# roahmlab/koopman-realizations

Hardware: AMD Instinct MI355X
Metric: EDMD snapshot-pairs/sec (bilinear fit, 3-link arm, poly-3) (higher is better)
Workload: dtype f64

## Files before the change

### koopman-realizations_amd/csrc/kp_context.hip

```cpp
#include <algorithm>
#include <cmath>
#include <cstring>
#include <mutex>

#include "kp_internal.h"

static std::mutex g_err_mu;
static std::string g_err;

void kp_set_global_error(const std::string& s) {
  std::lock_guard<std::mutex> l(g_err_mu);
  g_err = s;
}

void* kp_ctx::workspace(int slot, size_t bytes) {
  if (ws_bytes[slot] >= bytes && ws[slot]) return ws[slot];
  if (ws[slot]) (void)hipFree(ws[slot]);
  ws[slot] = nullptr;
  ws_bytes[slot] = 0;
  size_t want = bytes + bytes / 4 + 256;
  if (hipMalloc(&ws[slot], want) != hipSuccess) return nullptr;
  ws_bytes[slot] = want;
  return ws[slot];
}
// ... 50 lines not shown
  (void)kp_flush_grams(c);
  (void)kp_comm_destroy(c);
  (void)hipSetDevice(c->device);
  kp_stage_destroy(c);
  (void)hipStreamSynchronize(c->stream);
  if (c->stream2) (void)hipStreamSynchronize(c->stream2);
  for (int i = 0; i < 21; ++i)
    if (c->ws[i]) (void)hipFree(c->ws[i]);
  if (c->sticky_info) (void)hipFree(c->sticky_info);
  if (c->pin_small) (void)hipHostFree(c->pin_small);
  if (c->pin_scratch) (void)hipHostFree(c->pin_scratch);
  if (c->ev_gram_done) (void)hipEventDestroy(c->ev_gram_done);
  if (c->ev_pad_done) (void)hipEventDestroy(c->ev_pad_done);
  if (c->ev_pad_done2) (void)hipEventDestroy(c->ev_pad_done2);
  if (c->ev_main_done) (void)hipEventDestroy(c->ev_main_done);
  if (c->ev_solve0) (void)hipEventDestroy(c->ev_solve0);
  if (c->ev_solve1) (void)hipEventDestroy(c->ev_solve1);
  if (c->stream2) (void)hipStreamDestroy(c->stream2);
  if (c->Kres) (void)hipFree(c->Kres);
  if (c->GC) (void)hipFree(c->GC);
  for (int i = 0; i < 6; ++i)
    if (c->evp[i]) (void)hipEventDestroy(c->evp[i]);
  for (int i = 0; i < 2 * 64; ++i)
    if (c->ring[i]) (void)hipEventDestroy(c->ring[i]);
  for (int i = 0; i < 64; ++i)
    if (c->ring_red[i]) (void)hipEventDestroy(c->ring_red[i]);
  (void)hipEventDestroy(c->ev0);
  (void)hipEventDestroy(c->ev1);
  (void)hipStreamDestroy(c->stream);
  kp_traj_pool_free(c);
  kp_host_free_all(c);
  delete c;
  return KP_OK;
}

extern "C" int kp_device_count(int* count) {
  if (!count) return KP_ERR_ARG;
  int n = 0;
  if (hipGetDeviceCount(&n) != hipSuccess) {
    (void)hipGetLastError();
    n = 0;
  }
  *count = n;
  return KP_OK;
}

extern "C" const char* kp_last_error(const kp_ctx* c) {
  if (c) return c->err.c_str();
  std::lock_guard<std::mutex> l(g_err_mu);
  static thread_local std::string copy;
  copy = g_err;
  return copy.c_str();
}

extern "C" int kp_device_info(const kp_ctx* c, char* name, int name_len, int* num_cu, int64_t* hbm) {
  if (!c) return KP_ERR_ARG;
  if (name && name_len > 0) {
    std::strncpy(name, c->name.c_str(), (size_t)name_len - 1);
    name[name_len - 1] = 0;
  }
  if (num_cu) *num_cu = c->num_cu;
  if (hbm) *hbm = c->hbm_bytes;
  return KP_OK;
}

void* kp_pinned_scratch(kp_ctx* ctx, size_t bytes) {
  if (ctx->pin_scratch_bytes >= bytes) return ctx->pin_scratch;
  if (ctx->pin_scratch) {
    (void)hipStreamSynchronize(ctx->stream);
    (void)hipHostFree(ctx->pin_scratch);
  }
  ctx->pin_scratch = nullptr;
  ctx->pin_scratch_bytes = 0;
  const size_t cap = (bytes + 4095) & ~(size_t)4095;
  if (hipHostMalloc(&ctx->pin_scratch, cap, hipHostMallocDefault) != hipSuccess) {
    ctx->pin_scratch = nullptr;
    return nullptr;
  }
  ctx->pin_scratch_bytes = cap;
  return ctx->pin_scratch;
}

extern "C" int kp_timer_get(const kp_ctx* c, int which, double* ms) {
  if (!c || !ms || which < 0 || which >= 15) return KP_ERR_ARG;
  *ms = c->timers[which];
  return KP_OK;
}

extern "C" void* kp_stream(const kp_ctx* c) { return c ? (void*)c->stream : nullptr; }


static int upload(kp_ctx* ctx, void** dst, const void* src, size_t bytes) {
  *dst = nullptr;
  if (bytes == 0) return KP_OK;
  KP_HIP(ctx, hipMalloc(dst, bytes));
  KP_HIP(ctx, hipMemcpy(*dst, src, bytes, hipMemcpyHostToDevice));
  return KP_OK;
}

extern "C" int kp_basis_desc_dims(const kp_basis_desc* d, int* nvars_out, int* nfull_out, int* N_out, int* W_out) {
  if (!d || d->nzeta < 1 || d->m < 0 || d->model_type < 0 || d->model_type > 2 || d->n_blocks < 0 ||
      (d->n_blocks && (!d->block_type || !d->block_count)))
    return KP_ERR_ARG;
  const int nvars = d->nzeta + (d->model_type == KP_MODEL_NONLINEAR ? d->m : 0);
  double nf = nvars + 1.0;
  for (int b = 0; b < d->n_blocks; ++b) {
    const int c = d->block_count[b];
    if (c < 0) return KP_ERR_ARG;
    switch (d->block_type[b]) {
      case KP_BLOCK_POLY: case KP_BLOCK_HERMITE: case KP_BLOCK_FOURIER_SPARSER: case KP_BLOCK_GAUSSIAN: nf += c; break;
      case KP_BLOCK_FOURIER: nf += std::pow((double)(2 * c + 1), (double)nvars) - 1.0; break;
      default: return KP_ERR_ARG;
    }
    if (nf > 1e6) return KP_ERR_ARG;
  }
  const int nfull = (int)std::llround(nf);
  const int N = d->k_pcs > 0 ? d->k_pcs + nvars + 1 : nfull;
  if (nvars_out) *nvars_out = nvars;
  if (nfull_out) *nfull_out = nfull;
  if (N_out) *N_out = N;
  if (W_out) *W_out = d->model_type == KP_MODEL_BILINEAR ? N * (d->m + 1) : d->model_type == KP_MODEL_LINEAR ? N + d->m : N;
  return KP_OK;
}

extern "C" int kp_basis_create(kp_ctx* ctx, const kp_basis_desc* d, kp_basis** out) {
  if (!ctx || !d || !out) return KP_ERR_ARG;
  *out = nullptr;
  KP_HIP(ctx, hipSetDevice(ctx->device));
  if (d->model_type < 0 || d->model_type > 2) return ctx->fail(KP_ERR_ARG, "kp_basis_create: model_type");
  if (d->nzeta < 1 || d->m < 0) return ctx->fail(KP_ERR_ARG, "kp_basis_create: nzeta/m");
  int nvars = d->nzeta + (d->model_type == KP_MODEL_NONLINEAR ? d->m : 0);
  if (nvars > KP_MAX_VARS) return ctx->fail(KP_ERR_ARG, "kp_basis_create: too many variables (max 32)");
  std::vector<ColDesc> cols;
  for (int i = 0; i < nvars; ++i) cols.push_back({COL_VAR, i, 0, 0});
  int n_mono = 0, n_gauss = 0, max_deg = 1, fourier_deg = 0;
  for (int b = 0; b < d->n_blocks; ++b) {
    int cnt = d->block_count[b];
    if (cnt < 0) return ctx->fail(KP_ERR_ARG, "kp_basis_create: negative block count");
    switch (d->block_type[b]) {
      case KP_BLOCK_POLY:
        if (cnt && !d->poly_exps) return ctx->fail(KP_ERR_ARG, "kp_basis_create: poly_exps is NULL");
        for (int i = 0; i < cnt; ++i) {
          int deg = 0;
          for (int v = 0; v < nvars; ++v) deg += d->poly_exps[(size_t)(n_mono + i) * nvars + v];
          if (deg > max_deg) max_deg = deg;
          uint32_t pk[2] = {0, 0};
          if (nvars <= 8)
            for (int v = 0; v < nvars; ++v) pk[v >> 2] |= (uint32_t)d->poly_exps[(size_t)(n_mono + i) * nvars + v] << (8 * (v & 3));
          cols.push_back({COL_MONO, n_mono + i, (int32_t)pk[0], (int32_t)pk[1]});
        }
        n_mono += cnt;
        break;
      case KP_BLOCK_FOURIER: {
        if (cnt < 1) return ctx->fail(KP_ERR_ARG, "kp_basis_create: fourier degree < 1");
        double nf = std::pow((double)(2 * cnt + 1), (double)nvars);
        if (nf > 1e6) return ctx->fail(KP_ERR_ARG, "kp_basis_create: fourier block too large");
        int total = (int)std::llround(nf);
        for (int i = 1; i < total; ++i) {
          uint32_t pk = 0;
          if (nvars <= 8 && 2 * cnt + 1 <= 16) {
            int idx = i;
            for (int v = nvars - 1; v >= 0; --v) {
              pk |= (uint32_t)(idx % (2 * cnt + 1)) << (4 * v);
              idx /= 2 * cnt + 1;
            }
          }
          cols.push_back({COL_FOURIER, i, cnt, (int32_t)pk});
// ... 380 lines not shown
```

### koopman-realizations_amd/csrc/kp_gram3.hip

```cpp
#include <algorithm>
#include <cstdlib>
#include <type_traits>
#include <vector>

#include "kp_internal.h"

#ifndef KP_RAW_STEP
#define KP_RAW_STEP 1
#endif
#define KT3 8
#define NF3 3
#define RS3 240
#define YOFF3 96
#define ZOFF3 192
#define WOFF3 196
#define SOFF3 208
#define NIDMAX3 144
#define PST3 10
#define POWBUF3 (PST3 * NIDMAX3)
#define PSIBUF3 (KT3 * RS3)
#define PSI03 (2 * POWBUF3)
#define LDS3_DOUBLES (PSI03 + 2 * PSIBUF3)
#define PCS03 LDS3_DOUBLES
#define PCSMAX3 32
// ... 507 lines not shown
    default: run_tiles(std::integral_constant<int, NQ>{}); break;
  }

  double* dst = a.part + (((size_t)split * a.njobs + job) * NQ) * NWT * 64 + lane;
#pragma unroll
  for (int q = 0; q < NQ; ++q)
#pragma unroll
    for (int w = 0; w < NWT; ++w) dst[(q * NWT + w) * 64] = acc[q][w];
}

__global__ __launch_bounds__(1024) void kp_gram3_reduce_kernel(const double* __restrict__ part, int nsplit, int njobs, int NQ, int NWT,
                                                              int BM, const uint32_t* __restrict__ desc, int G4, int N, int W,
                                                              double* __restrict__ G, double* __restrict__ C, int tup,
                                                              const uint32_t* __restrict__ dst_off, const uint32_t* __restrict__ dst) {
  const int idx = blockIdx.x;
  int w = idx % NWT;
  const int jq = idx / NWT, q = jq % NQ, job = jq / NQ;
  const int l = threadIdx.x & 63, wv = threadIdx.x >> 6, nwv = blockDim.x >> 6;
  __shared__ double red[16][64];
  const size_t per_split = (size_t)njobs * NQ * NWT * 64;
  const double* src = part + (size_t)blockIdx.y * nsplit * per_split + (size_t)idx * 64 + l;
  G += (size_t)blockIdx.y * 2 * W * W;
  C += (size_t)blockIdx.y * 2 * W * W;
  double s0 = 0.0, s1 = 0.0, s2 = 0.0, s3 = 0.0;
  int p = wv;
  for (; p + 3 * nwv < nsplit; p += 4 * nwv) {
    const double v0 = src[(size_t)p * per_split], v1 = src[(size_t)(p + nwv) * per_split];
    const double v2 = src[(size_t)(p + 2 * nwv) * per_split], v3 = src[(size_t)(p + 3 * nwv) * per_split];
    s0 += v0; s1 += v1; s2 += v2; s3 += v3;
  }
  for (; p < nsplit; p += nwv) s0 += src[(size_t)p * per_split];
  red[wv][l] = (s0 + s1) + (s2 + s3);
  __syncthreads();
  if (wv) return;
  double s = red[0][l];
  for (int v = 1; v < nwv; ++v) s += red[v][l];
  const uint32_t* jd = desc + (size_t)job * (1 + NQ);
  const int ga = q < (int)((jd[0] >> 16) & 255u) ? (int)(jd[0] & 255u) : (int)((jd[0] >> 8) & 255u);
  int gsel = (l >> 2) & 3;
  if (tup) {
    const int b = gsel;
    gsel = 2 * (w & 1) + (b & 1);
    w = (w & ~1) + (b >> 1);
  }
  const int gb = (int)((jd[1 + q] >> (8 * gsel)) & 255u);
  if (gb >= 2 * G4) return;
  int wa = 0, wb = 0, cnt = 0;
  for (int x = 0; x <= BM; ++x)
    for (int y = x; y <= BM; ++y) {
      if (cnt == w) { wa = x; wb = y; }
      ++cnt;
    }
  const int ia = 4 * ga + (l >> 4);
  if (ia >= N) return;
  if (gb < G4 && dst_off) {
    const int e = (jq * 4 + gsel) * 16 + (l >> 4) * 4 + (l & 3);
    for (uint32_t k = dst_off[e]; k < dst_off[e + 1]; ++k) {
      const uint32_t d = dst[k];
      const size_t di = d & 0xffffu, dj = d >> 16;
      const size_t r1 = (size_t)wa * N + di, c1 = (size_t)wb * N + dj;
      const size_t r2 = (size_t)wb * N + di, c2 = (size_t)wa * N + dj;
      G[c1 * W + r1] = s; G[r1 * W + c1] = s;
      G[c2 * W + r2] = s; G[r2 * W + c2] = s;
    }
  } else if (gb < G4) {
    const int jb = 4 * gb + (l & 3);
    if (jb >= N) return;
    if (ga == gb && ia > jb) return;
    const size_t r1 = (size_t)wa * N + ia, c1 = (size_t)wb * N + jb;
    const size_t r2 = (size_t)wb * N + ia, c2 = (size_t)wa * N + jb;
    G[c1 * W + r1] = s; G[r1 * W + c1] = s;
    G[c2 * W + r2] = s; G[r2 * W + c2] = s;
  } else {
    const int jb = 4 * (gb - G4) + (l & 3);
    if (jb >= N) return;
    C[((size_t)wb * N + jb) * W + (size_t)wa * N + ia] = s;
    C[((size_t)wa * N + jb) * W + (size_t)wb * N + ia] = s;
  }
}

struct kp_gram3_plan {
  int G4 = 0, nq = 0, njobs = 0, nsuper = 0;
  int wpw = 4;
  uint32_t* desc = nullptr;
  uint32_t* dst_off = nullptr;
  uint32_t* dst = nullptr;
  kp_gram3_plan* cover = nullptr;
  bool cover_tried = false;
};

void kp_gram3_plan_free(kp_gram3_plan* p) {
  if (!p) return;
  kp_gram3_plan_free(p->cover);
  if (p->desc) (void)hipFree(p->desc);
  if (p->dst_off) (void)hipFree(p->dst_off);
  if (p->dst) (void)hipFree(p->dst);
  delete p;
}

static hipError_t plan3_upload(uint32_t** dev, const std::vector<uint32_t>& host) {
  hipError_t e = hipMalloc((void**)dev, std::max<size_t>(host.size(), 1) * 4);
  if (e == hipSuccess && !host.empty()) e = hipMemcpy(*dev, host.data(), host.size() * 4, hipMemcpyHostToDevice);
  return e;
}

static int make_plan3(kp_ctx* ctx, int N, int nwt, int nq_cap, kp_gram3_plan** out, int wpw = 4, int nq_force = 0) {
  kp_gram3_plan* p = new kp_gram3_plan();
  p->wpw = wpw;
  const int G4 = (N + 3) / 4;
  p->G4 = G4;
  size_t maxq = 0;
  const std::vector<std::vector<int>> rows = gram3_circulant_rows(G4, &maxq);
  Gram3JobsHost jobs;
  gram3_pack_rows(rows, G4, nwt, nq_cap, maxq, wpw, nq_force, &jobs);
  p->nq = jobs.nq;
  p->njobs = jobs.njobs;
  p->nsuper = jobs.njobs / wpw;
  hipError_t e = plan3_upload(&p->desc, jobs.desc);
  if (e != hipSuccess) {
    kp_gram3_plan_free(p);
    return ctx->fail(KP_ERR_HIP, std::string("kp_fit_gram: plan upload: ") + hipGetErrorString(e));
  }
  *out = p;
  return KP_OK;
}

static bool gram3_tup(int bm) {
  static const bool off = getenv("KP_GRAM3_NOTUP") != nullptr;
  return bm >= 2 && !off;
}

template <int NQ, int BM, bool PCS, bool EXT = false, bool PRE = false, bool TUP = false>
static hipError_t launch3c(const Gram3Args& a, int grid, size_t lds, hipStream_t st) {
  static KpLdsCache lds_cache;
  {
    const size_t lds_max = (size_t)(LDS3_DOUBLES + (PCS ? LDS3_PCS_DOUBLES : 0) + (EXT ? LDS3_GAUSS_DOUBLES : 0)) * sizeof(double);
    hipError_t e = kp_ensure_lds(lds_cache, (const void*)kp_gram3_kernel<NQ, BM, PCS, EXT, PRE, TUP>, lds_max);
    if (e != hipSuccess) return e;
  }
  hipLaunchKernelGGL((kp_gram3_kernel<NQ, BM, PCS, EXT, PRE, TUP>), dim3(grid), dim3(256), lds, st, a);
  return hipGetLastError();
}

template <int NQ, int BM, bool PCS, bool EXT = false, bool PRE = false>
static hipError_t launch3b(const Gram3Args& a, int grid, size_t lds, hipStream_t st) {
  if constexpr (BM >= 2) {
    if (gram3_tup(BM)) return launch3c<NQ, BM, PCS, EXT, PRE, true>(a, grid, lds, st);
  }
  return launch3c<NQ, BM, PCS, EXT, PRE, false>(a, grid, lds, st);
}

template <int NQ>
static hipError_t launch3(const Gram3Args& a, int bm, int grid, size_t lds, hipStream_t st) {
  if (a.pre) {
    switch (bm) {
      case 1: return launch3b<NQ, 1, false, false, true>(a, grid, lds, st);
      case 2: return launch3b<NQ, 2, false, false, true>(a, grid, lds, st);
      default: return launch3b<NQ, 3, false, false, true>(a, grid, lds, st);
    }
  }
  if (a.pcs) {
    if constexpr (NQ <= 4) {
      switch (bm) {
        case 1: return launch3b<NQ, 1, true>(a, grid, lds, st);
        case 2: return launch3b<NQ, 2, true>(a, grid, lds, st);
        default: return launch3b<NQ, 3, true>(a, grid, lds, st);
      }
    } else {
      return hipErrorInvalidValue;
    }
  }
  if (a.df > 0 || a.ng > 0) {
    switch (bm) {
      case 1: return launch3b<NQ, 1, false, true>(a, grid, lds, st);
      case 2: return launch3b<NQ, 2, false, true>(a, grid, lds, st);
      default: return launch3b<NQ, 3, false, true>(a, grid, lds, st);
    }
  }
  switch (bm) {
    case 1: return launch3b<NQ, 1, false>(a, grid, lds, st);
    case 2: return launch3b<NQ, 2, false>(a, grid, lds, st);
    default: return launch3b<NQ, 3, false>(a, grid, lds, st);
  }
}

static bool gram3_ext(const kp_basis* basis) {
  const BasisDev& b = basis->dev;
  return basis->fast_ext && (basis->ext_df > 0 || basis->ext_ng > 0) && b.k_pcs == 0 && basis->ext_ng <= GAUSSMAX3 &&
         (basis->ext_ng == 0 || b.nzeta <= GNZMAX3) && !getenv("KP_NO_GRAM3_EXT");
}

static bool gram3_prelift(const kp_basis* basis) {
  static const bool off = getenv("KP_GRAM3_NO_PRELIFT") != nullptr;
  const BasisDev& b = basis->dev;
  if (off) return false;
  if ((b.N + 3) / 4 > 14) return false;
  if (b.k_pcs > 0) return b.k_pcs <= 32 && basis->fast && b.nzeta * basis->pow_depth <= 24;
  return gram3_ext(basis) && b.nzeta <= 16 && b.nzeta * (basis->ext_Dp + 2 * basis->ext_df) + basis->ext_ng + 1 <= 64;
}

bool kp_gram3_applicable(const kp_basis* basis) {
  const BasisDev& b = basis->dev;
  if (getenv("KP_NO_GRAM3")) return false;
  if (2 * b.nfull + (b.m + 1) * (b.m + 2) / 2 - 1 > 192) return false;
  if (gram3_ext(basis))
    return b.model_type == KP_MODEL_BILINEAR && basis->ext_max_factors <= NF3 && b.nfull <= YOFF3 && b.m >= 1 && b.m <= 3 &&
           2 * (b.nzeta + b.m) * KT3 <= 256 &&
           2 * (b.nzeta + b.m) * (basis->ext_Dp + 2 * basis->ext_df) + 1 + 2 * basis->ext_ng <= NIDMAX3;
  if (b.k_pcs > 0 && (b.k_pcs > PCSMAX3 || b.N != b.nzeta + b.k_pcs + 1 || getenv("KP_NO_GRAM3_PCS"))) return false;
  return b.model_type == KP_MODEL_BILINEAR && basis->fast && basis->max_factors <= NF3 && b.nfull <= YOFF3 && basis->pow_depth <= 4 &&
         b.m >= 1 && b.m <= 3 && (2 * (b.nzeta + b.m) + 1) * KT3 <= 256 && 2 * (b.nzeta + b.m) * 4 + 4 <= NIDMAX3;
}

static bool gram6_on() {
  static const bool on = getenv("KP_GRAM6") != nullptr;
  return on;
}

static int gram3_plan(kp_ctx* ctx, kp_basis* basis) {
  if (basis->plan3) return KP_OK;
  const BasisDev& b = basis->dev;
  const int N = b.N, BM = b.m, NWT = (BM + 1) * (BM + 2) / 2;
  static const int ext_cap = [] { const char* e = getenv("KP_GRAM3_EXT_NQ"); return e ? atoi(e) : 4; }();
  const bool g6 = gram6_on() && BM == 3 && b.k_pcs == 0 && !gram3_ext(basis) && kp_gram6_serves(7, (N + 3) / 4);
  return g6 ? make_plan3(ctx, N, NWT, 7, &basis->plan3, 8, 7)
            : make_plan3(ctx, N, NWT, b.k_pcs > 0 ? 4 : gram3_ext(basis) ? ext_cap : 6, &basis->plan3);
}

static int gram3_cover_mode() {
  static const int v = [] { const char* e = getenv("KP_GRAM3_COVER"); return e ? std::min(2, std::max(0, atoi(e))) : 1; }();
  return v;
}

static int gram3_cover_plan(kp_ctx* ctx, kp_basis* basis, kp_gram3_plan** out) {
  kp_gram3_plan& circ = *basis->plan3;
  *out = nullptr;
  if (!circ.cover_tried) {
    circ.cover_tried = true;
    const BasisDev& b = basis->dev;
    const int N = b.N, NWT = (b.m + 1) * (b.m + 2) / 2;
    if (circ.wpw != 4 || b.k_pcs != 0 || gram3_ext(basis) || !basis->fast || b.nfull != N || (int)basis->h_recipes.size() != N) return KP_OK;
    Gram3CoverHost cov;
    if (!gram3_cover_build(basis->h_recipes.data(), N, basis->pow_depth, NWT, 6, circ.wpw, &cov) || cov.jobs.njobs >= circ.njobs) return KP_OK;
    kp_gram3_plan* p = new kp_gram3_plan();
    p->G4 = circ.G4;
    p->nq = cov.jobs.nq;
    p->njobs = cov.jobs.njobs;
    p->nsuper = cov.jobs.njobs / circ.wpw;
    p->cover_tried = true;
    hipError_t e = plan3_upload(&p->desc, cov.jobs.desc);
    if (e == hipSuccess) e = plan3_upload(&p->dst_off, cov.dst_off);
    if (e == hipSuccess) e = plan3_upload(&p->dst, cov.dst);
    if (e != hipSuccess) {
      kp_gram3_plan_free(p);
      circ.cover_tried = false;
      return ctx->fail(KP_ERR_HIP, std::string("kp_fit_gram: plan upload: ") + hipGetErrorString(e));
    }
    circ.cover = p;
  }
  *out = circ.cover;
  return KP_OK;
}

static int gram3_plan_for(kp_ctx* ctx, kp_basis* basis, bool deferred, kp_gram3_plan** out) {
  int rc = gram3_plan(ctx, basis);
  if (rc) return rc;
  *out = basis->plan3;
  if (gram3_cover_mode() == 2 || (gram3_cover_mode() == 1 && deferred)) {
    kp_gram3_plan* cov = nullptr;
    rc = gram3_cover_plan(ctx, basis, &cov);
    if (rc) return rc;
    if (cov) *out = cov;
  }
  return KP_OK;
}

static int64_t gram3_slots(const kp_ctx* ctx, const kp_gram3_plan& plan, int* ncu_out = nullptr, int* wgpcu_out = nullptr) {
  int ncu = ctx->num_cu > 0 ? ctx->num_cu : 256;
  int wg_per_cu = plan.wpw == 8 ? 1 : 2;
  if (const char* ov = getenv("KP_GRAM3_WGPCU")) wg_per_cu = std::max(1, atoi(ov));
  if (ncu_out) *ncu_out = ncu;
  if (wgpcu_out) *wgpcu_out = wg_per_cu;
  return (int64_t)std::max(8, ncu - ctx->reserve_cus) * wg_per_cu;
}

bool kp_gram3_groupable(kp_ctx* ctx, const kp_basis* basis_c, const kp_snapshots* s) {
  kp_basis* basis = const_cast<kp_basis*>(basis_c);
  const BasisDev& b = basis->dev;
  if (!(kp_gram3_applicable(basis) && b.k_pcs == 0 && !gram3_ext(basis) && !gram6_on() && s->nzeta == b.nzeta && s->m == b.m)) return false;
  kp_gram3_plan* plan = nullptr;
  if (gram3_plan_for(ctx, basis, true, &plan) != KP_OK || plan->wpw == 8) return false;
  static const int64_t max_kps = [] { const char* e = getenv("KP_GRAM_GROUP_MAX_KPS"); return e ? (int64_t)atoll(e) : (int64_t)512; }();
  const int64_t ktiles = (s->Ns + KT3 - 1) / KT3, nsplit = std::max<int64_t>(1, gram3_slots(ctx, *plan) / plan->nsuper);
  return (ktiles + nsplit - 1) / nsplit < max_kps;
}

static int gram3_launch_n(kp_ctx* ctx, const kp_basis* basis_c, const kp_snapshots* const* ss, int n, double* GC_dev, bool cover) {
  kp_basis* basis = const_cast<kp_basis*>(basis_c);
  const BasisDev& b = basis->dev;
  const kp_snapshots* s = ss[0];
  if (n < 1 || n > KP_GRAM_GROUP_MAX) return ctx->fail(KP_ERR_ARG, "kp_fit_gram: bad group size");
  for (int f = 0; f < n; ++f)
    if (ss[f]->nzeta != b.nzeta || ss[f]->m != b.m || ss[f]->Ns != s->Ns) return ctx->fail(KP_ERR_ARG, "kp_fit_gram: snapshot/basis dimension mismatch");
  const int W = b.W, N = b.N;
  const int BM = b.m, NWT = (BM + 1) * (BM + 2) / 2;
  kp_gram3_plan* planp = nullptr;
  {
    int rc = gram3_plan_for(ctx, basis, cover, &planp);
    if (rc) return rc;
  }
  kp_gram3_plan& plan = *planp;
  const int nfull4 = (b.nfull + 3) / 4 * 4;
  const bool ext = gram3_ext(basis);
  
  int64_t ktiles = (s->Ns + KT3 - 1) / KT3;
  int ncu, wg_per_cu;
  const int64_t slots = gram3_slots(ctx, plan, &ncu, &wg_per_cu);
  int nsplit = (int)std::max<int64_t>(1, std::min<int64_t>(ktiles, slots / plan.nsuper / n > 0 ? slots / plan.nsuper / n : 1));
  int kps = (int)((ktiles + nsplit - 1) / nsplit);
  if (kps < 1) kps = 1;
  nsplit = (int)std::max<int64_t>(1, (ktiles + kps - 1) / kps);
  size_t per_split = (size_t)plan.njobs * plan.nq * NWT * 64;
  const size_t part_bytes = ((size_t)n * nsplit * per_split * 8 + 255) & ~(size_t)255;
  if (gram3_cover_mode() != 0) {
    kp_gram3_plan* cov = nullptr;
    int rc = gram3_cover_plan(ctx, basis, &cov);
    if (rc) return rc;
  }
// ... 24 lines not shown
  if (pre && !ext && !basis->d_pcsT) {
    if (hipMalloc(&basis->d_pcsT, (size_t)b.nfull * 32 * 8) != hipSuccess) return ctx->fail(KP_ERR_HIP, "kp_fit_gram: out of device memory");
    KP_HIP(ctx, kp_gram3_pcs_transpose_launch(b.pcs, b.nfull, b.k_pcs, (double*)basis->d_pcsT, ctx->stream));
  }
  const size_t lds = (size_t)(LDS3_DOUBLES + (b.k_pcs > 0 && !pre ? 2 * nfull4 * 16 : 0) + (ext && !pre ? LDS3_GAUSS_DOUBLES : 0)) * sizeof(double);

  Gram3Args a;
  a.b = b;
  a.alpha = s->alpha;
  a.beta = s->beta;
  a.u = s->u;
  a.Ns = s->Ns;
  a.G4 = plan.G4;
  a.nsuper = plan.nsuper;
  a.ktiles_per_split = kps;
  a.D = ext ? basis->ext_Dp + 2 * basis->ext_df : basis->pow_depth;
  a.recipes = (const uint32_t*)(ext ? basis->d_recipes_ext : basis->d_recipes);
  a.Dp = ext ? basis->ext_Dp : basis->pow_depth;
  a.df = ext ? basis->ext_df : 0;
  a.ng = ext ? basis->ext_ng : 0;
  a.centres = b.centres;
  a.desc = plan.desc;
  a.part = part;
  a.njobs = plan.njobs;
  a.pcs = b.k_pcs > 0 && !pre ? b.pcs : nullptr;
  a.nfull4 = nfull4;
  a.pre = pre_buf;
  a.pre_rl = pre_rl;
  a.nsplit_fit = nsplit;
  for (int f = 0; f < n; ++f) a.grp[f] = Gram3Src{ss[f]->alpha, ss[f]->beta, ss[f]->u};
  const int grid = plan.nsuper * nsplit * n;
  const bool pipelined = ctx->reduce_stream || ctx->ring_timing;
  if (!pipelined) KP_HIP(ctx, hipEventRecord(ctx->ev0, ctx->stream));
  hipEvent_t ev_start = ctx->evp[0], ev_end = ctx->evp[1];
  const bool timed = !ctx->ring_timing || (ctx->ring_group && n > 1) || (ctx->ring_skip++ & 3) == 0;
  hipEvent_t ev_red = nullptr;
  if (pipelined && timed) {
    ev_start = ctx->ring[2 * ctx->ring_pos];
    ev_end = ctx->ring[2 * ctx->ring_pos + 1];
    ctx->ring_members[ctx->ring_pos] = n;
    ctx->ring_has_red[ctx->ring_pos] = false;
    if (ctx->ring_timing && ctx->ring_group && n > 1) {
      ev_red = ctx->ring_red[ctx->ring_pos];
      ctx->ring_has_red[ctx->ring_pos] = ev_red != nullptr;
    }
    ctx->ring_pos = (ctx->ring_pos + 1) % 64;
    if (ctx->ring_n < 64) ++ctx->ring_n;
  }
  if (timed) KP_HIP(ctx, hipEventRecord(ev_start, ctx->stream));
  hipError_t e;
  if (pre && ext)
    KP_HIP(ctx, kp_gram3_prelift_ext_launch(BM, s->alpha, s->beta, s->u, s->Ns, ktiles * KT3, b.nzeta, basis->ext_Dp, basis->ext_df, basis->ext_ng, b.nfull, plan.G4,
                                            (const uint32_t*)basis->d_recipes_ext, b.centres, pre_buf, pre_rl, ctx->stream));
  else if (pre)
    KP_HIP(ctx, kp_gram3_prelift_launch(BM, s->alpha, s->beta, s->u, s->Ns, ktiles * KT3, b.nzeta, basis->pow_depth, b.nfull, b.k_pcs, N, plan.G4,
                                        (const uint32_t*)basis->d_recipes, (const double*)basis->d_pcsT, pre_buf, pre_rl, ctx->stream));
  if (plan.wpw == 8) e = kp_gram6_launch_kernel(a, plan.nq, grid, ctx->stream);
  else switch (plan.nq) {
    case 1: e = launch3<1>(a, BM, grid, lds, ctx->stream); break;
    case 2: e = launch3<2>(a, BM, grid, lds, ctx->stream); break;
    case 3: e = launch3<3>(a, BM, grid, lds, ctx->stream); break;
    case 4: e = launch3<4>(a, BM, grid, lds, ctx->stream); break;
    case 5: e = launch3<5>(a, BM, grid, lds, ctx->stream); break;
    default: e = launch3<6>(a, BM, grid, lds, ctx->stream); break;
  }
  KP_HIP(ctx, e);
  if (timed) KP_HIP(ctx, hipEventRecord(ev_end, ctx->stream));
  hipStream_t rs = ctx->stream;
  if (ctx->reduce_stream) {
    rs = ctx->reduce_stream;
    KP_HIP(ctx, hipStreamWaitEvent(rs, ev_end, 0));
    KP_HIP(ctx, hipEventRecord(ctx->evp[4], rs));
    ctx->solve_chained = true;
  }
  ctx->reduce_timed_from = ctx->reduce_stream ? 4 : 1;
  hipLaunchKernelGGL(kp_gram3_reduce_kernel, dim3(plan.njobs * plan.nq * NWT, n), dim3(nsplit >= 128 ? 1024 : nsplit >= 32 ? 512 : 256), 0, rs, part, nsplit, plan.njobs,
                     plan.nq, NWT, BM, plan.desc, plan.G4, N, W, GC_dev, GC_dev + (size_t)W * W, plan.wpw != 8 && gram3_tup(BM) ? 1 : 0, plan.dst_off, plan.dst);
  KP_HIP(ctx, hipGetLastError());
  if (ev_red) KP_HIP(ctx, hipEventRecord(ev_red, rs));
  if (!pipelined) KP_HIP(ctx, hipEventRecord(ctx->ev1, rs));
  if (!ctx->ring_timing) KP_HIP(ctx, hipEventRecord(ctx->evp[2], rs));
  ctx->gram_flops_per_pair = (double)W * (W + 1) + 2.0 * W * W;
  ctx->timers[10] = (double)plan.njobs * plan.nq * NWT * 128.0 + (b.k_pcs > 0 && !pre ? (double)plan.nsuper * nfull4 * 128.0 : 0.0);
  return KP_OK;
}

int kp_gram3_launch(kp_ctx* ctx, const kp_basis* basis, const kp_snapshots* s, double* GC_dev, bool cover) { return gram3_launch_n(ctx, basis, &s, 1, GC_dev, cover); }

int kp_gram3_launch_group(kp_ctx* ctx, const kp_basis* basis, const kp_snapshots* const* ss, int n, double* GC_dev) {
  return gram3_launch_n(ctx, basis, ss, n, GC_dev, true);
}


__global__ __launch_bounds__(256) void kp_gram3_linear_gather_kernel(const double* __restrict__ GCb, int N, int m, int Wb, double* __restrict__ GC) {
  const int W = N + m;
  const int e = blockIdx.x * 256 + threadIdx.x;
  if (e >= 2 * W * W) return;
  const int which = e / (W * W), r = e - which * W * W, i = r % W, j = r / W;
  const int bi = i < N ? i : (i - N + 1) * N + N - 1, bj = j < N ? j : (j - N + 1) * N + N - 1;
  GC[e] = GCb[(size_t)which * Wb * Wb + (size_t)bj * Wb + bi];
}

static kp_basis* gram3_shadow(const kp_basis* basis_c) {
  kp_basis* basis = const_cast<kp_basis*>(basis_c);
  if (!basis->shadow_bil) {
    kp_basis* sh = new kp_basis(*basis);
    sh->dev.model_type = KP_MODEL_BILINEAR;
    sh->dev.W = sh->dev.N * (sh->dev.m + 1);
    sh->plan = nullptr; sh->plan2 = nullptr; sh->plan3 = nullptr; sh->plan5 = nullptr; sh->shadow_bil = nullptr;
    sh->d_pcsT = nullptr;
    basis->shadow_bil = sh;
  }
  return basis->shadow_bil;
}

void kp_gram3_shadow_free(kp_basis* basis) {
  if (!basis) return;
  if (basis->shadow_bil) {
    kp_gram3_plan_free(basis->shadow_bil->plan3);
    if (basis->shadow_bil->d_pcsT) (void)hipFree(basis->shadow_bil->d_pcsT);
    delete basis->shadow_bil;
    basis->shadow_bil = nullptr;
  }
  if (basis->shadow_full) {
    kp_gram_plan_free(basis->shadow_full->plan);
    kp_gram2_plan_free(basis->shadow_full->plan2);
    kp_gram5_plan_free(basis->shadow_full->plan5);
    delete basis->shadow_full;
    basis->shadow_full = nullptr;
  }
}

bool kp_gram3_linear_applicable(const kp_basis* basis) {
  const BasisDev& b = basis->dev;
  if (b.model_type != KP_MODEL_LINEAR || b.k_pcs <= 0 || b.m < 1 || getenv("KP_NO_GRAM3_LINEAR")) return false;
  return kp_gram3_applicable(gram3_shadow(basis));
}

int kp_gram3_linear_launch(kp_ctx* ctx, const kp_basis* basis, const kp_snapshots* s, double* GC_dev) {
  kp_basis* sh = gram3_shadow(basis);
  const int N = basis->dev.N, m = basis->dev.m, W = basis->dev.W, Wb = sh->dev.W;
  double* tmp = (double*)ctx->workspace(10, (size_t)2 * Wb * Wb * 8);
  if (!tmp) return ctx->fail(KP_ERR_HIP, "kp_fit_gram: out of device memory");
  hipStream_t rs = ctx->reduce_stream ? ctx->reduce_stream : ctx->stream;
  int rc = kp_gram3_launch(ctx, sh, s, tmp);
  if (rc) return rc;
  hipLaunchKernelGGL(kp_gram3_linear_gather_kernel, dim3((2 * W * W + 255) / 256), dim3(256), 0, rs, tmp, N, m, Wb, GC_dev);
  KP_HIP(ctx, hipGetLastError());
  ctx->gram_flops_per_pair = (double)W * (W + 1) + 2.0 * W * W;
  return KP_OK;
}


struct CongT { int nvars, k, nfull, N, W, Wf; const double* pcs; };
__device__ __forceinline__ int cong_unit(const CongT& t, int j) {
  if (j < t.nvars) return j;
  if (j < t.nvars + t.k) return -1;
  if (j == t.N - 1) return t.nfull - 1;
  return t.nfull + (j - t.N);
}
__global__ __launch_bounds__(256) void kp_cong_right_kernel(const double* __restrict__ GCf, CongT t, double* __restrict__ R) {
  const int e = blockIdx.x * 256 + threadIdx.x;
  if (e >= t.Wf * t.W) return;
  const int i = e % t.Wf, j = e / t.Wf;
  const double* M = GCf + (size_t)blockIdx.y * t.Wf * t.Wf;
  const int u = cong_unit(t, j);
// ... 77 lines not shown
```

### koopman-realizations_amd/csrc/kp_gram3_cover.h

```cpp
#pragma once
#include <algorithm>
#include <cstdint>
#include <cstdlib>
#include <map>
#include <utility>
#include <vector>

struct Gram3JobsHost {
  int nq = 0, njobs = 0, nquads = 0;
  std::vector<uint32_t> desc;
};

inline std::vector<std::vector<int>> gram3_circulant_rows(int G4, size_t* maxq) {
  std::vector<std::vector<int>> rows(G4);
  *maxq = 0;
  for (int g = 0; g < G4; ++g) {
    for (int d = 0; d <= G4 / 2; ++d) {
      if (d > 0 && 2 * d == G4 && g >= G4 / 2) continue;
      rows[g].push_back((g + d) % G4);
    }
    for (int h = 0; h < G4; ++h) rows[g].push_back(G4 + h);
    *maxq = std::max(*maxq, (rows[g].size() + 3) / 4);
  }
  return rows;
// ... 104 lines not shown

  std::vector<std::vector<int>> rows(G4);
  for (auto& p : chosen)
    if (p.first == p.second) rows[p.first].push_back(p.second);
  std::vector<std::pair<int, int>> off;
  for (auto& p : chosen)
    if (p.first != p.second) off.push_back(p);
  std::sort(off.begin(), off.end());
  auto quads_of = [&](size_t s) { return (s + G4 + 3) / 4; };
  for (auto& p : off) {
    const size_t la = rows[p.first].size(), lb = rows[p.second].size();
    const size_t ca = quads_of(la + 1) - quads_of(la), cb = quads_of(lb + 1) - quads_of(lb);
    const bool to_b = cb < ca || (cb == ca && lb < la);
    rows[to_b ? p.second : p.first].push_back(to_b ? p.first : p.second);
  }
  size_t minq = ~(size_t)0;
  for (int g = 0; g < G4; ++g) {
    for (int h = 0; h < G4; ++h) rows[g].push_back(G4 + h);
    minq = std::min(minq, (rows[g].size() + 3) / 4);
  }
  gram3_pack_rows(rows, G4, nwt, nq_cap, minq, wpw, 0, &out->jobs);
  out->npairs = (int)chosen.size();
  out->nmonos = nm;

  const Gram3JobsHost& J = out->jobs;
  const int nq = J.nq;
  std::vector<int> src(nm, -1);
  std::vector<int> tgroups((size_t)G4 * G4, 0);
  for (int job = 0; job < J.njobs; ++job) {
    const uint32_t* jd = &J.desc[(size_t)job * (1 + nq)];
    const int a0 = (int)(jd[0] & 255u), a1 = (int)((jd[0] >> 8) & 255u), qs = (int)((jd[0] >> 16) & 255u);
    if (a0 >= G4 || a1 >= G4) return false;
    for (int q = 0; q < nq; ++q) {
      const int ga = q < qs ? a0 : a1;
      for (int k = 0; k < 4; ++k) {
        const int gb = (int)((jd[1 + q] >> (8 * k)) & 255u);
        if (gb > 2 * G4) return false;
        if (gb >= G4) {
          if (gb < 2 * G4) ++tgroups[(size_t)ga * G4 + gb - G4];
          continue;
        }
        for (int r = 0; r < 4; ++r)
          for (int c = 0; c < 4; ++c) {
            const int i = 4 * ga + r, j = 4 * gb + c;
            if (i >= N || j >= N) continue;
            int& s = src[mono[(size_t)i * N + j]];
            if (s < 0) s = ((job * nq + q) * 4 + k) * 16 + 4 * r + c;
          }
      }
    }
  }
  for (int t : tgroups)
    if (t != 1) return false;
  const int nel = J.njobs * nq * 64;
  std::vector<uint32_t> cnt(nel + 1, 0);
  for (int i = 0; i < N; ++i)
    for (int j = i; j < N; ++j) {
      const int s = src[mono[(size_t)i * N + j]];
      if (s < 0) return false;
      ++cnt[s + 1];
    }
  for (int e = 0; e < nel; ++e) cnt[e + 1] += cnt[e];
  out->dst_off = cnt;
  out->dst.assign(cnt[nel], 0);
  std::vector<uint32_t> fill(cnt.begin(), cnt.end() - 1);
  for (int i = 0; i < N; ++i)
    for (int j = i; j < N; ++j) out->dst[fill[src[mono[(size_t)i * N + j]]]++] = (uint32_t)i | ((uint32_t)j << 16);
  if ((size_t)cnt[nel] != (size_t)N * (N + 1) / 2) return false;
  for (int e = 0; e < nel; ++e) {
    if (cnt[e] == cnt[e + 1]) continue;
    const int c = e & 3, r = (e >> 2) & 3, k = (e >> 4) & 3, jq = e >> 6, q = jq % nq, job = jq / nq;
    const uint32_t* jd = &J.desc[(size_t)job * (1 + nq)];
    const int ga = q < (int)((jd[0] >> 16) & 255u) ? (int)(jd[0] & 255u) : (int)((jd[0] >> 8) & 255u);
    const int gb = (int)((jd[1 + q] >> (8 * k)) & 255u);
    const int i = 4 * ga + r, j = 4 * gb + c;
    if (gb >= G4 || i >= N || j >= N) return false;
    for (uint32_t d = cnt[e]; d < cnt[e + 1]; ++d) {
      const int di = (int)(out->dst[d] & 0xffffu), dj = (int)(out->dst[d] >> 16);
      if (di > dj || dj >= N || mono[(size_t)di * N + dj] != mono[(size_t)i * N + j]) return false;
    }
  }
  return true;
}
```

### koopman-realizations_amd/csrc/kp_internal.h

```cpp
#pragma once
#include <hip/hip_runtime.h>
#include <stdint.h>
#include <atomic>
#include <mutex>
#include <string>
#include <utility>
#include <vector>

#include "koopman_hip.h"

#define KP_MAX_VARS 32
#define KP_GRAM_GROUP_MAX 8

void kp_set_global_error(const std::string& s);
void kp_traj_device_blocks(kp_traj* t, double** blocks);
struct kp_comm_state;

struct kp_stage;

struct kp_ctx {
  int device = 0;
  kp_stage* stage = nullptr;
  std::vector<void*> host_blocks;
  std::vector<std::pair<void*, size_t>> traj_pool;
  std::mutex host_mu;
  hipStream_t stream = nullptr;
  hipEvent_t ev0 = nullptr, ev1 = nullptr;
  hipEvent_t evp[6] = {nullptr};
  hipStream_t stream2 = nullptr;
  hipEvent_t ev_gram_done = nullptr, ev_pad_done = nullptr, ev_pad_done2 = nullptr, ev_solve0 = nullptr, ev_solve1 = nullptr;
  bool pad_pending = false, pad_pending2 = false, async_pending = false;
  int gc_flip = 0;
  int kring_cap = 128;
  int async_count = 0;
  bool batch_closed = true;
  bool kres_is_ring = false;
  const void* pend_basis = nullptr;
  int64_t pend_Ns = 0;
  int pend_W = 0;
  int pend_solves = 0, pend_first = 0;
  bool ring_timing = false;
  unsigned ring_skip = 0;
  const kp_snapshots* pend_grams[KP_GRAM_GROUP_MAX] = {};
  int pend_ngrams = 0;
  const kp_basis* pend_gram_basis = nullptr;
  double* pend_gram_gc = nullptr;
  bool ring_group = false;
  kp_comm_state* comm = nullptr;
  std::atomic<bool> comm_abandoned{false};
  bool gc_preloaded = false;
  bool reduce_grams = false;
  hipStream_t reduce_stream = nullptr;
  hipEvent_t ev_main_done = nullptr;
  hipEvent_t ring[2 * 64] = {};
  int ring_pos = 0, ring_n = 0;
  hipEvent_t ring_red[64] = {};
  int ring_members[64] = {};
  bool ring_has_red[64] = {};
  bool solve_chained = false;
  int part_flip = 0;
  int reduce_timed_from = 1;
  int* sticky_info = nullptr;
  bool test_hooks = false;
  void* pin_scratch = nullptr;
  size_t pin_scratch_bytes = 0;
  double* pin_small = nullptr;
  int reserve_cus = 0;
  int num_cu = 0;
  int64_t hbm_bytes = 0;
  std::string name;
  mutable std::string err;
  double timers[15] = {0};
  double gram_flops_per_pair = 0;
  void* ws[21] = {nullptr};
  size_t ws_bytes[21] = {0};
  int last_rank = -1;
  double last_pivot_ratio = 1.0;
  double* Kres = nullptr;
  size_t Kres_bytes = 0;
  int Kres_W = 0, Kres_n = 0;
  double* GC = nullptr;
  size_t GC_bytes = 0;
  int GC_W = 0;

  int fail(int code, const std::string& s) const {
    err = s;
    kp_set_global_error(s);
    return code;
  }
  void* workspace(int slot, size_t bytes);
};

#define KP_HIP(ctx, expr)                                                                  \
  do {                                                                                     \
    hipError_t _e = (expr);                                                                \
    if (_e != hipSuccess)                                                                  \
      return (ctx)->fail(KP_ERR_HIP, std::string(#expr) + ": " + hipGetErrorString(_e));   \
  } while (0)

enum : int { COL_VAR = 0, COL_MONO = 1, COL_FOURIER = 2, COL_GAUSS = 3, COL_CONST = 4, COL_HERMITE = 5, COL_FSPARSE = 6 };

struct ColDesc {
  int32_t kind;
  int32_t arg;
  int32_t aux;
  int32_t pad;
};

struct BasisDev {
  int model_type, nzeta, m, nvars;
  int nfull, N, W, k_pcs;
  const ColDesc* cols;
  const uint8_t* exps;
  const double* centres;
  const double* pcs;
};

struct KpLdsCache { size_t set[32] = {}; };
inline hipError_t kp_ensure_lds(KpLdsCache& c, const void* func, size_t lds) {
  int dev = -1;
  if (hipGetDevice(&dev) != hipSuccess || dev < 0 || dev >= 32) return hipFuncSetAttribute(func, hipFuncAttributeMaxDynamicSharedMemorySize, (int)lds);
  if (lds > c.set[dev]) {
    hipError_t e = hipFuncSetAttribute(func, hipFuncAttributeMaxDynamicSharedMemorySize, (int)lds);
    if (e != hipSuccess) return e;
    c.set[dev] = lds;
  }
  return hipSuccess;
}

struct kp_gram_plan;
void kp_gram_plan_free(kp_gram_plan* p);
struct kp_gram2_plan;
void kp_gram2_plan_free(kp_gram2_plan* p);
struct kp_gram3_plan;
void kp_gram3_plan_free(kp_gram3_plan* p);
struct kp_gram5_plan;
void kp_gram5_plan_free(kp_gram5_plan* p);

struct kp_basis {
  kp_ctx* ctx = nullptr;
  BasisDev dev{};
  void* d_cols = nullptr;
  void* d_exps = nullptr;
  void* d_centres = nullptr;
  void* d_pcs = nullptr;
  void* d_recipes = nullptr;
  void* d_pcsT = nullptr;
  int max_degree = 0;
  mutable int rank_hint = 0;
  bool pure_fourier = false;
  int fourier_degree = 0;
  int pow_depth = 1;
  bool fast = false;
  int max_factors = 1;
  kp_gram_plan* plan = nullptr;
// ... 179 lines not shown
```

Baseline: 312.4 million.

## Build one-row-group Gram cover plan with hub rows to avoid split jobs

Adds a host-side builder that re-packs the monomial cover plan so every Gram job handles a single row group, with a few hub rows allowed two jobs. The builder searches hub sets greedily until every distinct monomial is covered. It replaces the existing cover plan when job count and quads per job stay the same, removing two-group jobs, whose mixed rows likely cost extra loads or divergence in the kernel. It also records the number of two-group jobs in a new timer slot, and adds host planning cost that can reach up to 2048 hub-set trials.

After: 324.6 million (median of 6 runs). 1.04x the previous value.

```diff
diff --git a/koopman-realizations_amd/csrc/kp_context.hip b/koopman-realizations_amd/csrc/kp_context.hip
--- a/koopman-realizations_amd/csrc/kp_context.hip
+++ b/koopman-realizations_amd/csrc/kp_context.hip
@@ -156,7 +156,7 @@
 }
 
 extern "C" int kp_timer_get(const kp_ctx* c, int which, double* ms) {
-  if (!c || !ms || which < 0 || which >= 15) return KP_ERR_ARG;
+  if (!c || !ms || which < 0 || which >= 16) return KP_ERR_ARG;
   *ms = c->timers[which];
   return KP_OK;
 }
diff --git a/koopman-realizations_amd/csrc/kp_gram3.hip b/koopman-realizations_amd/csrc/kp_gram3.hip
--- a/koopman-realizations_amd/csrc/kp_gram3.hip
+++ b/koopman-realizations_amd/csrc/kp_gram3.hip
@@ -613,6 +613,7 @@
 struct kp_gram3_plan {
   int G4 = 0, nq = 0, njobs = 0, nsuper = 0;
   int wpw = 4;
+  int two_group_jobs = 0;
   uint32_t* desc = nullptr;
   uint32_t* dst_off = nullptr;
   uint32_t* dst = nullptr;
@@ -647,6 +648,7 @@
   p->nq = jobs.nq;
   p->njobs = jobs.njobs;
   p->nsuper = jobs.njobs / wpw;
+  p->two_group_jobs = gram3_two_group_jobs(jobs);
   hipError_t e = plan3_upload(&p->desc, jobs.desc);
   if (e != hipSuccess) {
     kp_gram3_plan_free(p);
@@ -763,6 +765,11 @@
   return v;
 }
 
+static bool gram3_onea_on() {
+  static const bool on = [] { const char* e = getenv("KP_GRAM3_ONEA"); return !e || atoi(e) != 0; }();
+  return on;
+}
+
 static int gram3_cover_plan(kp_ctx* ctx, kp_basis* basis, kp_gram3_plan** out) {
   kp_gram3_plan& circ = *basis->plan3;
   *out = nullptr;
@@ -773,8 +780,13 @@
     if (circ.wpw != 4 || b.k_pcs != 0 || gram3_ext(basis) || !basis->fast || b.nfull != N || (int)basis->h_recipes.size() != N) return KP_OK;
     Gram3CoverHost cov;
     if (!gram3_cover_build(basis->h_recipes.data(), N, basis->pow_depth, NWT, 6, circ.wpw, &cov) || cov.jobs.njobs >= circ.njobs) return KP_OK;
+    if (gram3_onea_on()) {
+      Gram3CoverHost one;
+      if (gram3_onea_build(basis->h_recipes.data(), N, basis->pow_depth, cov, &one) && one.jobs.nq == cov.jobs.nq && one.jobs.njobs <= cov.jobs.njobs) cov = std::move(one);
+    }
     kp_gram3_plan* p = new kp_gram3_plan();
     p->G4 = circ.G4;
+    p->two_group_jobs = gram3_two_group_jobs(cov.jobs);
     p->nq = cov.jobs.nq;
     p->njobs = cov.jobs.njobs;
     p->nsuper = cov.jobs.njobs / circ.wpw;
@@ -965,6 +977,7 @@
   if (!ctx->ring_timing) KP_HIP(ctx, hipEventRecord(ctx->evp[2], rs));
   ctx->gram_flops_per_pair = (double)W * (W + 1) + 2.0 * W * W;
   ctx->timers[10] = (double)plan.njobs * plan.nq * NWT * 128.0 + (b.k_pcs > 0 && !pre ? (double)plan.nsuper * nfull4 * 128.0 : 0.0);
+  ctx->timers[15] = (double)plan.two_group_jobs;
   return KP_OK;
 }
 
diff --git a/koopman-realizations_amd/csrc/kp_gram3_cover.h b/koopman-realizations_amd/csrc/kp_gram3_cover.h
--- a/koopman-realizations_amd/csrc/kp_gram3_cover.h
+++ b/koopman-realizations_amd/csrc/kp_gram3_cover.h
@@ -210,3 +210,249 @@
   }
   return true;
 }
+
+
+inline int gram3_monomial_ids(const uint32_t* recipes, int N, int D, std::vector<int>* mono) {
+  if (N < 1 || D < 1 || N > 4 * 127) return 0;
+  int nv = 1;
+  for (int c = 0; c < N; ++c)
+    for (int f = 0; f < 4; ++f) {
+      const int id = (int)((recipes[c] >> (8 * f)) & 255u);
+      if (id != 255) nv = std::max(nv, id / D + 1);
+    }
+  std::vector<std::vector<uint8_t>> ex(N, std::vector<uint8_t>(nv, 0));
+  for (int c = 0; c < N; ++c)
+    for (int f = 0; f < 4; ++f) {
+      const int id = (int)((recipes[c] >> (8 * f)) & 255u);
+      if (id != 255) ex[c][id / D] += (uint8_t)(id % D + 1);
+    }
+  std::map<std::vector<uint8_t>, int> ids;
+  mono->assign((size_t)N * N, 0);
+  std::vector<uint8_t> sum(nv);
+  for (int i = 0; i < N; ++i)
+    for (int j = 0; j < N; ++j) {
+      for (int v = 0; v < nv; ++v) sum[v] = (uint8_t)(ex[i][v] + ex[j][v]);
+      (*mono)[(size_t)i * N + j] = ids.emplace(sum, (int)ids.size()).first->second;
+    }
+  return (int)ids.size();
+}
+
+inline bool gram3_cover_sources(const std::vector<int>& mono, int nm, int N, bool one_group, Gram3CoverHost* out) {
+  const int G4 = (N + 3) / 4;
+  const Gram3JobsHost& J = out->jobs;
+  const int nq = J.nq;
+  if (nq < 1 || J.njobs < 1 || J.desc.size() != (size_t)J.njobs * (1 + nq)) return false;
+  std::vector<int> src(nm, -1);
+  std::vector<int> tgroups((size_t)G4 * G4, 0);
+  for (int job = 0; job < J.njobs; ++job) {
+    const uint32_t* jd = &J.desc[(size_t)job * (1 + nq)];
+    const int a0 = (int)(jd[0] & 255u), a1 = (int)((jd[0] >> 8) & 255u), qs = (int)((jd[0] >> 16) & 255u);
+    if (a0 >= G4 || a1 >= G4) return false;
+    if (one_group && (qs != nq || a1 != a0)) return false;
+    for (int q = 0; q < nq; ++q) {
+      const int ga = q < qs ? a0 : a1;
+      for (int k = 0; k < 4; ++k) {
+        const int gb = (int)((jd[1 + q] >> (8 * k)) & 255u);
+        if (gb > 2 * G4) return false;
+        if (gb >= G4) {
+          if (gb < 2 * G4) ++tgroups[(size_t)ga * G4 + gb - G4];
+          continue;
+        }
+        for (int r = 0; r < 4; ++r)
+          for (int c = 0; c < 4; ++c) {
+            const int i = 4 * ga + r, j = 4 * gb + c;
+            if (i >= N || j >= N) continue;
+            int& s = src[mono[(size_t)i * N + j]];
+            if (s < 0) s = ((job * nq + q) * 4 + k) * 16 + 4 * r + c;
+          }
+      }
+    }
+  }
+  for (int t : tgroups)
+    if (t != 1) return false;
+  const int nel = J.njobs * nq * 64;
+  std::vector<uint32_t> cnt(nel + 1, 0);
+  for (int i = 0; i < N; ++i)
+    for (int j = i; j < N; ++j) {
+      const int s = src[mono[(size_t)i * N + j]];
+      if (s < 0) return false;
+      ++cnt[s + 1];
+    }
+  for (int e = 0; e < nel; ++e) cnt[e + 1] += cnt[e];
+  out->dst_off = cnt;
+  out->dst.assign(cnt[nel], 0);
+  std::vector<uint32_t> fill(cnt.begin(), cnt.end() - 1);
+  for (int i = 0; i < N; ++i)
+    for (int j = i; j < N; ++j) out->dst[fill[src[mono[(size_t)i * N + j]]]++] = (uint32_t)i | ((uint32_t)j << 16);
+  if ((size_t)cnt[nel] != (size_t)N * (N + 1) / 2) return false;
+  for (int e = 0; e < nel; ++e) {
+    if (cnt[e] == cnt[e + 1]) continue;
+    const int c = e & 3, r = (e >> 2) & 3, k = (e >> 4) & 3, jq = e >> 6, q = jq % nq, job = jq / nq;
+    const uint32_t* jd = &J.desc[(size_t)job * (1 + nq)];
+    const int ga = q < (int)((jd[0] >> 16) & 255u) ? (int)(jd[0] & 255u) : (int)((jd[0] >> 8) & 255u);
+    const int gb = (int)((jd[1 + q] >> (8 * k)) & 255u);
+    const int i = 4 * ga + r, j = 4 * gb + c;
+    if (gb >= G4 || i >= N || j >= N) return false;
+    for (uint32_t d = cnt[e]; d < cnt[e + 1]; ++d) {
+      const int di = (int)(out->dst[d] & 0xffffu), dj = (int)(out->dst[d] >> 16);
+      if (di > dj || dj >= N || mono[(size_t)di * N + dj] != mono[(size_t)i * N + j]) return false;
+    }
+  }
+  return true;
+}
+
+inline int gram3_two_group_jobs(const Gram3JobsHost& J) {
+  int n = 0;
+  for (int job = 0; job < J.njobs; ++job) n += (int)((J.desc[(size_t)job * (1 + J.nq)] >> 16) & 255u) < J.nq;
+  return n;
+}
+
+constexpr int GRAM3_ONEA_MAX_SETS = 2048;
+
+inline bool gram3_onea_build(const uint32_t* recipes, int N, int D, const Gram3CoverHost& cover, Gram3CoverHost* out, std::vector<int>* hubs = nullptr) {
+  std::vector<int> mono;
+  const int nm = gram3_monomial_ids(recipes, N, D, &mono);
+  if (nm < 1 || nm != cover.nmonos) return false;
+  const int G4 = (N + 3) / 4, ZG = 2 * G4, nq = cover.jobs.nq, njobs = cover.jobs.njobs;
+  const int H = njobs - G4, cap_light = 4 * nq - G4, cap_hub = 8 * nq - G4;
+  if (gram3_two_group_jobs(cover.jobs) == 0) return false;
+  if (H < 0 || H > G4 || cap_light < 0) return false;
+
+  const int NP = G4 * (G4 + 1) / 2;
+  std::vector<int> pa(NP), pb(NP), pcnt(NP, 0), pmono((size_t)NP * 16);
+  {
+    int p = 0;
+    for (int ga = 0; ga < G4; ++ga)
+      for (int gb = ga; gb < G4; ++gb, ++p) {
+        pa[p] = ga;
+        pb[p] = gb;
+        int* mine = &pmono[(size_t)p * 16];
+        for (int r = 0; r < 4; ++r)
+          for (int c = 0; c < 4; ++c) {
+            if (4 * ga + r >= N || 4 * gb + c >= N) continue;
+            const int mo = mono[(size_t)(4 * ga + r) * N + 4 * gb + c];
+            if (std::find(mine, mine + pcnt[p], mo) == mine + pcnt[p]) mine[pcnt[p]++] = mo;
+          }
+      }
+  }
+  std::vector<int> moff(nm + 1, 0), mpair;
+  for (int p = 0; p < NP; ++p)
+    for (int k = 0; k < pcnt[p]; ++k) ++moff[pmono[(size_t)p * 16 + k] + 1];
+  for (int mo = 0; mo < nm; ++mo) moff[mo + 1] += moff[mo];
+  mpair.resize(moff[nm]);
+  {
+    std::vector<int> fill(moff.begin(), moff.end() - 1);
+    for (int p = 0; p < NP; ++p)
+      for (int k = 0; k < pcnt[p]; ++k) mpair[fill[pmono[(size_t)p * 16 + k]]++] = p;
+  }
+
+  std::vector<int> hub(H);
+  for (int h = 0; h < H; ++h) hub[h] = h;
+  std::vector<int> gain(NP), cap(G4), act(NP), hact(NP);
+  std::vector<char> have(nm), is_hub(G4);
+  std::vector<std::vector<int>> srow(G4);
+  bool found = false;
+  for (int tried = 0; tried < GRAM3_ONEA_MAX_SETS && !found; ++tried) {
+    std::fill(is_hub.begin(), is_hub.end(), 0);
+    for (int h : hub) is_hub[h] = 1;
+    for (int g = 0; g < G4; ++g) {
+      cap[g] = is_hub[g] ? cap_hub : cap_light;
+      srow[g].clear();
+    }
+    gain = pcnt;
+    std::fill(have.begin(), have.end(), 0);
+    int left = nm;
+    int nact = NP, nhact = 0;
+    for (int p = 0; p < NP; ++p) {
+      act[p] = p;
+      if (is_hub[pa[p]] || is_hub[pb[p]]) hact[nhact++] = p;
+    }
+    while (left > 0) {
+      int best = -1, bgain = 0, keep = 0;
+      for (int x = 0; x < nhact; ++x) {
+        const int p = hact[x], ga = pa[p], gb = pb[p];
+        if (gain[p] == 0 || !((is_hub[ga] && cap[ga] > 0) || (is_hub[gb] && cap[gb] > 0))) continue;
+        hact[keep++] = p;
+        if (gain[p] > bgain) { bgain = gain[p]; best = p; }
+      }
+      nhact = keep;
+      if (best < 0) {
+        keep = 0;
+        for (int x = 0; x < nact; ++x) {
+          const int p = act[x], ga = pa[p], gb = pb[p];
+          if (gain[p] == 0 || (cap[ga] <= 0 && cap[gb] <= 0)) continue;
+          act[keep++] = p;
+          if (gain[p] > bgain) { bgain = gain[p]; best = p; }
+        }
+        nact = keep;
+      }
+      if (best < 0) break;
+      const int ga = pa[best], gb = pb[best];
+      const int ka = cap[ga] > 0 ? (is_hub[ga] ? 1024 : 0) + cap[ga] : -1, kb = cap[gb] > 0 ? (is_hub[gb] ? 1024 : 0) + cap[gb] : -1;
+      const bool to_b = kb > ka;
+      const int row = to_b ? gb : ga;
+      srow[row].push_back(to_b ? ga : gb);
+      --cap[row];
+      for (int k = 0; k < pcnt[best]; ++k) {
+        const int mo = pmono[(size_t)best * 16 + k];
+        if (have[mo]) continue;
+        have[mo] = 1;
+        --left;
+        for (int x = moff[mo]; x < moff[mo + 1]; ++x) --gain[mpair[x]];
+      }
+      bool dead = false;
+      for (int g = 0; cap[row] == 0 && g < G4 && !dead; ++g) {
+        if (cap[g] > 0) continue;
+        const int lo = std::min(g, row), hi = std::max(g, row), p = lo * G4 - lo * (lo - 1) / 2 + hi - lo;
+        for (int k = 0; k < pcnt[p] && !dead; ++k) {
+          const int mo = pmono[(size_t)p * 16 + k];
+          if (have[mo]) continue;
+          dead = true;
+          for (int x = moff[mo]; x < moff[mo + 1] && dead; ++x) dead = cap[pa[mpair[x]]] <= 0 && cap[pb[mpair[x]]] <= 0;
+        }
+      }
+      if (dead) break;
+    }
+    if (left == 0) { found = true; break; }
+    int h = H - 1;
+    while (h >= 0 && hub[h] == G4 - H + h) --h;
+    if (h < 0) break;
+    ++hub[h];
+    for (int k = h + 1; k < H; ++k) hub[k] = hub[k - 1] + 1;
+  }
+  if (!found) return false;
+
+  Gram3JobsHost& J = out->jobs;
+  J.nq = nq;
+  J.njobs = 0;
+  J.nquads = 0;
+  J.desc.clear();
+  int npairs = 0;
+  for (int g = 0; g < G4; ++g) {
+    std::vector<int> slots;
+    for (int h = 0; h < G4; ++h) slots.push_back(G4 + h);
+    slots.insert(slots.end(), srow[g].begin(), srow[g].end());
+    npairs += (int)srow[g].size();
+    const int jobs_g = is_hub[g] ? 2 : 1;
+    if ((int)slots.size() > jobs_g * 4 * nq) return false;
+    J.nquads += ((int)slots.size() + 3) / 4;
+    for (int jb = 0; jb < jobs_g; ++jb) {
+      J.desc.push_back((uint32_t)g | ((uint32_t)g << 8) | ((uint32_t)nq << 16));
+      for (int q = 0; q < nq; ++q) {
+        uint32_t packed = 0;
+        for (int k = 0; k < 4; ++k) {
+          const size_t idx = (size_t)(jb * nq + q) * 4 + k;
+          packed |= (uint32_t)(idx < slots.size() ? slots[idx] : ZG) << (8 * k);
+        }
+        J.desc.push_back(packed);
+      }
+      ++J.njobs;
+    }
+  }
+  if (J.njobs != njobs) return false;
+  out->npairs = npairs;
+  out->nmonos = nm;
+  if (!gram3_cover_sources(mono, nm, N, true, out)) return false;
+  if (hubs) *hubs = hub;
+  return true;
+}
diff --git a/koopman-realizations_amd/csrc/kp_internal.h b/koopman-realizations_amd/csrc/kp_internal.h
--- a/koopman-realizations_amd/csrc/kp_internal.h
+++ b/koopman-realizations_amd/csrc/kp_internal.h
@@ -70,7 +70,7 @@
   int64_t hbm_bytes = 0;
   std::string name;
   mutable std::string err;
-  double timers[15] = {0};
+  double timers[16] = {0};
   double gram_flops_per_pair = 0;
   void* ws[21] = {nullptr};
   size_t ws_bytes[21] = {0};
```
